# stanfordnlp/mac-network

Hardware: NVIDIA H100
Metric: mac_reasoning_steps_per_sec (higher is better)
Workload: dtype bf16

## Files before the change

mac_network_b200/csrc/read_step.cuh:

```cuda
#pragma once
#include "tc_gemm.cuh"

namespace mac {

constexpr int RS_D = 512;
constexpr int RS_BM = 64;
constexpr int RS_KB = RS_D / TC_BK;
constexpr int RS_BLK = RS_BM * TC_BK * 2;
constexpr int RS_A_BYTES = RS_KB * RS_BLK;
constexpr int RS_B_HALF = 256 * TC_BK * 2;
constexpr int RS_W_BYTES = 2 * RS_B_HALF;
constexpr int RS_STAGE = RS_W_BYTES + RS_BLK;
constexpr int RS_STAGES = 2;
constexpr int RS_Q_SLOT = RS_KB;
constexpr int RS_SLOTS = RS_Q_SLOT + 1 + RS_KB;
constexpr int RS_CONSUMERS = 256;
constexpr int RS_THREADS = RS_CONSUMERS + 32;
constexpr int RS_SMEM_BYTES = RS_A_BYTES + RS_STAGES * RS_STAGE + 1024  + 64  +
                              2 * RS_BM * 4  + 2 * RS_D * 4  +
                              2 * RS_D * 4 ;
static_assert(RS_SMEM_BYTES <= 232448, "over the sm_90 per-block shared memory opt-in limit");
static_assert(RS_STAGE % 1024 == 0 && RS_W_BYTES % 1024 == 0, "swizzled operands need 1024-byte alignment");

__device__ __forceinline__ float bf16lo(uint32_t w) { return __uint_as_float(w << 16); }
__device__ __forceinline__ float bf16hi(uint32_t w) { return __uint_as_float(w & 0xffff0000u); }

__device__ __forceinline__ void wgmma_bf16_n256(float (&d)[128], uint64_t adesc, uint64_t bdesc, uint32_t accum) {
  asm volatile(
      "{\n\t.reg .pred p;\n\t"
      "setp.ne.b32 p, %130, 0;\n\t"
      "wgmma.mma_async.sync.aligned.m64n256k16.f32.bf16.bf16 "
      "{%0, %1, %2, %3, %4, %5, %6, %7, %8, %9, %10, %11, %12, %13, %14, %15, %16, %17, %18, %19, %20, %21, %22, %23, %24, %25, %26, %27, %28, %29, %30, %31, %32, %33, %34, %35, %36, %37, %38, %39, %40, %41, %42, %43, %44, %45, %46, %47, %48, %49, %50, %51, %52, %53, %54, %55, %56, %57, %58, %59, %60, %61, %62, %63, %64, %65, %66, %67, %68, %69, %70, %71, %72, %73, %74, %75, %76, %77, %78, %79, %80, %81, %82, %83, %84, %85, %86, %87, %88, %89, %90, %91, %92, %93, %94, %95, %96, %97, %98, %99, %100, %101, %102, %103, %104, %105, %106, %107, %108, %109, %110, %111, %112, %113, %114, %115, %116, %117, %118, %119, %120, %121, %122, %123, %124, %125, %126, %127}, %128, %129, p, 1, 1, 0, 0;\n\t}"
      : "+f"(d[0]), "+f"(d[1]), "+f"(d[2]), "+f"(d[3]), "+f"(d[4]), "+f"(d[5]), "+f"(d[6]), "+f"(d[7]), "+f"(d[8]), "+f"(d[9]), "+f"(d[10]), "+f"(d[11]), "+f"(d[12]), "+f"(d[13]), "+f"(d[14]), "+f"(d[15]), "+f"(d[16]), "+f"(d[17]), "+f"(d[18]), "+f"(d[19]), "+f"(d[20]), "+f"(d[21]), "+f"(d[22]), "+f"(d[23]), "+f"(d[24]), "+f"(d[25]), "+f"(d[26]), "+f"(d[27]), "+f"(d[28]), "+f"(d[29]), "+f"(d[30]), "+f"(d[31]), "+f"(d[32]), "+f"(d[33]), "+f"(d[34]), "+f"(d[35]), "+f"(d[36]), "+f"(d[37]), "+f"(d[38]), "+f"(d[39]), "+f"(d[40]), "+f"(d[41]), "+f"(d[42]), "+f"(d[43]), "+f"(d[44]), "+f"(d[45]), "+f"(d[46]), "+f"(d[47]), "+f"(d[48]), "+f"(d[49]), "+f"(d[50]), "+f"(d[51]), "+f"(d[52]), "+f"(d[53]), "+f"(d[54]), "+f"(d[55]), "+f"(d[56]), "+f"(d[57]), "+f"(d[58]), "+f"(d[59]), "+f"(d[60]), "+f"(d[61]), "+f"(d[62]), "+f"(d[63]), "+f"(d[64]), "+f"(d[65]), "+f"(d[66]), "+f"(d[67]), "+f"(d[68]), "+f"(d[69]), "+f"(d[70]), "+f"(d[71]), "+f"(d[72]), "+f"(d[73]), "+f"(d[74]), "+f"(d[75]), "+f"(d[76]), "+f"(d[77]), "+f"(d[78]), "+f"(d[79]), "+f"(d[80]), "+f"(d[81]), "+f"(d[82]), "+f"(d[83]), "+f"(d[84]), "+f"(d[85]), "+f"(d[86]), "+f"(d[87]), "+f"(d[88]), "+f"(d[89]), "+f"(d[90]), "+f"(d[91]), "+f"(d[92]), "+f"(d[93]), "+f"(d[94]), "+f"(d[95]), "+f"(d[96]), "+f"(d[97]), "+f"(d[98]), "+f"(d[99]), "+f"(d[100]), "+f"(d[101]), "+f"(d[102]), "+f"(d[103]), "+f"(d[104]), "+f"(d[105]), "+f"(d[106]), "+f"(d[107]), "+f"(d[108]), "+f"(d[109]), "+f"(d[110]), "+f"(d[111]), "+f"(d[112]), "+f"(d[113]), "+f"(d[114]), "+f"(d[115]), "+f"(d[116]), "+f"(d[117]), "+f"(d[118]), "+f"(d[119]), "+f"(d[120]), "+f"(d[121]), "+f"(d[122]), "+f"(d[123]), "+f"(d[124]), "+f"(d[125]), "+f"(d[126]), "+f"(d[127])
      : "l"(adesc), "l"(bdesc), "r"(accum));
}
inline bool read_step_supported(int B, int N, int d) {
  return d == RS_D && N >= 1 && N <= 256 && B >= 1 && B < (1 << 22);
}

struct ReadStepParams {
  int M, N;
  const float* y;
  const float* ctrl;
  const float* bm2;
  const float* wr;
  float* logits;
};

__device__ __forceinline__ void rs_consumer_bar() { asm volatile("bar.sync 1, %0;" ::"n"(RS_CONSUMERS) : "memory"); }

__global__ void __launch_bounds__(RS_THREADS, 1)
read_step_kernel(const __grid_constant__ CUtensorMap map_p, const __grid_constant__ CUtensorMap map_q,
                 const __grid_constant__ CUtensorMap map_w1, const __grid_constant__ CUtensorMap map_w2,
                 const ReadStepParams p) {
  extern __shared__ unsigned char smem_dyn[];
  const uint32_t base_u32 = smem_u32(smem_dyn);
  unsigned char* a_tile = smem_dyn + ((1024u - (base_u32 & 1023u)) & 1023u);
  unsigned char* b_ring = a_tile + RS_A_BYTES;
  uint64_t* full = reinterpret_cast<uint64_t*>(b_ring + RS_STAGES * RS_STAGE);
  uint64_t* empty = full + RS_STAGES;
  float* s_lg = reinterpret_cast<float*>(full + 8);
  float* s_ctrl = s_lg + 2 * RS_BM;
  float* s_bm2 = s_ctrl + 2 * RS_D;
  float* s_wr = s_bm2 + RS_D;

  const int warp = threadIdx.x >> 5, lane = threadIdx.x & 31;
  const int row0 = blockIdx.x * RS_BM;
  const int s_lo = row0 / p.N;

  if (threadIdx.x == RS_CONSUMERS) {
    tma_prefetch_desc(&map_p);
    tma_prefetch_desc(&map_q);
    tma_prefetch_desc(&map_w1);
    tma_prefetch_desc(&map_w2);
    for (int i = 0; i < RS_STAGES; ++i) {
      mbar_init(&full[i], 1);
      mbar_init(&empty[i], RS_CONSUMERS / 32);
    }
    fence_mbar_init();
  }
  __syncthreads();

  if (warp == RS_CONSUMERS / 32) {
    if (elect_one()) {
      for (int j = 0; j < RS_SLOTS; ++j) {
        const int s = j % RS_STAGES;
        mbar_wait(&empty[s], ((j / RS_STAGES) & 1) ^ 1);
        unsigned char* dst = b_ring + s * RS_STAGE;
        if (j == RS_Q_SLOT) {
          mbar_expect_tx(&full[s], RS_A_BYTES);
          for (int kb = 0; kb < RS_KB; ++kb) tma_load_2d(dst + kb * RS_BLK, &map_q, kb * TC_BK, row0, &full[s]);
          continue;
        }
        const bool g1 = j < RS_Q_SLOT;
        mbar_expect_tx(&full[s], g1 ? RS_W_BYTES + RS_BLK : RS_W_BYTES);
        const CUtensorMap* m = g1 ? &map_w1 : &map_w2;
        const int k0 = (g1 ? j : j - RS_Q_SLOT - 1) * TC_BK;
        if (g1) tma_load_2d(dst + RS_W_BYTES, &map_p, k0, row0, &full[s]);
        tma_load_2d(dst, m, k0, 0, &full[s]);
        tma_load_2d(dst + RS_B_HALF, m, k0, 256, &full[s]);
      }
    }
    return;
  }

  const int tid = threadIdx.x;
  const int g = warp >> 2;
  const int rl = 16 * (warp & 3) + (lane >> 2);
  const int cq = 256 * g + 2 * (lane & 3);
  const int prow = tid >> 3;
  const int poff = prow * 128 + (tid & 7) * 16;
  const int pcol = ((tid & 7) ^ (prow & 7)) << 3;
  for (int i = tid; i < RS_D; i += RS_CONSUMERS) {
    s_bm2[i] = __ldg(p.bm2 + i);
    s_wr[i] = __ldg(p.wr + i);
  }
  float acc[128];
  const int last_row = min(p.M, row0 + RS_BM) - 1;
  const int nsamp = last_row / p.N - s_lo + 1;
  for (int q = 0; q < min(nsamp, 2); ++q)
    for (int i = tid; i < RS_D; i += RS_CONSUMERS) s_ctrl[q * RS_D + i] = __ldg(p.ctrl + (size_t)(s_lo + q) * RS_D + i);
  int yoff[2];
#pragma unroll
  for (int u = 0; u < 2; ++u) yoff[u] = min(row0 + prow + 32 * u, p.M - 1) / p.N * RS_D + pcol;

  for (int j = 0; j < RS_KB; ++j) {
    const int s = j % RS_STAGES;
    unsigned char* stage = b_ring + s * RS_STAGE;
    float4 y0[2], y1[2];
#pragma unroll
    for (int u = 0; u < 2; ++u) {
      y0[u] = *reinterpret_cast<const float4*>(p.y + yoff[u] + j * TC_BK);
      y1[u] = *reinterpret_cast<const float4*>(p.y + yoff[u] + j * TC_BK + 4);
    }
    mbar_wait(&full[s], (j / RS_STAGES) & 1);
#pragma unroll
    for (int u = 0; u < 2; ++u) {
      uint4* c = reinterpret_cast<uint4*>(stage + RS_W_BYTES + poff + u * 32 * 128);
      const uint4 v = *c;
      *c = make_uint4(pack_bf16(bf16lo(v.x) * y0[u].x, bf16hi(v.x) * y0[u].y), pack_bf16(bf16lo(v.y) * y0[u].z, bf16hi(v.y) * y0[u].w),
                      pack_bf16(bf16lo(v.z) * y1[u].x, bf16hi(v.z) * y1[u].y), pack_bf16(bf16lo(v.w) * y1[u].z, bf16hi(v.w) * y1[u].w));
    }
    fence_proxy_async();
    rs_consumer_bar();
    const uint64_t adesc = make_sw128_kmajor_desc(smem_u32(stage + RS_W_BYTES));
    const uint64_t bdesc = make_sw128_kmajor_desc(smem_u32(stage + g * RS_B_HALF));
    wgmma_fence();
#pragma unroll
    for (int k = 0; k < TC_BK / 16; ++k) wgmma_bf16_n256(acc, adesc + 2 * k, bdesc + 2 * k, (j || k) ? 1u : 0u);
    wgmma_commit();
    wgmma_wait<1>();
    wgmma_hold(acc);
    if (j && lane == 0) mbar_arrive(&empty[(j - 1) % RS_STAGES]);
  }
  wgmma_wait<0>();
  wgmma_hold(acc);
  if (lane == 0) mbar_arrive(&empty[(RS_KB - 1) % RS_STAGES]);

  constexpr int qs = RS_Q_SLOT % RS_STAGES;
  const unsigned char* q_tile = b_ring + qs * RS_STAGE;
  mbar_wait(&full[qs], (RS_Q_SLOT / RS_STAGES) & 1);
#pragma unroll
  for (int h = 0; h < 2; ++h) {
    const int r = rl + 8 * h, row = row0 + r;
#pragma unroll
    for (int j = 0; j < 32; ++j) {
      const int n = cq + 8 * j;
      const int kb = n >> 6, c = (n & 63) >> 3;
      const int off = kb * RS_BLK + r * 128 + ((c ^ (r & 7)) << 4) + (n & 7) * 2;
      const uint32_t q = *reinterpret_cast<const uint32_t*>(q_tile + off);
      const uint32_t hv = row < p.M ? pack_bf16(elu_fast(acc[4 * j + 2 * h] + bf16lo(q)), elu_fast(acc[4 * j + 2 * h + 1] + bf16hi(q)))
                                    : 0u;
      *reinterpret_cast<uint32_t*>(a_tile + off) = hv;
    }
  }
  fence_proxy_async();
  rs_consumer_bar();
  if (lane == 0) mbar_arrive(&empty[qs]);

  const uint32_t a_u = smem_u32(a_tile);
  for (int j = 0; j < RS_KB; ++j) {
    const int jj = RS_Q_SLOT + 1 + j, s = jj % RS_STAGES;
    mbar_wait(&full[s], (jj / RS_STAGES) & 1);
    const uint64_t adesc = make_sw128_kmajor_desc(a_u + j * RS_BLK);
    const uint64_t bdesc = make_sw128_kmajor_desc(smem_u32(b_ring + s * RS_STAGE + g * RS_B_HALF));
    wgmma_fence();
#pragma unroll
    for (int k = 0; k < TC_BK / 16; ++k) wgmma_bf16_n256(acc, adesc + 2 * k, bdesc + 2 * k, (j || k) ? 1u : 0u);
    wgmma_commit();
    wgmma_wait<1>();
    wgmma_hold(acc);
    if (j && lane == 0) mbar_arrive(&empty[(jj - 1) % RS_STAGES]);
  }
  wgmma_wait<0>();
  wgmma_hold(acc);
  if (lane == 0) mbar_arrive(&empty[(RS_SLOTS - 1) % RS_STAGES]);

#pragma unroll
  for (int h = 0; h < 2; ++h) {
    const int r = rl + 8 * h, row = row0 + r;
    const int s = min(row, p.M - 1) / p.N;
    const float* crow = s - s_lo < 2 ? s_ctrl + (s - s_lo) * RS_D : p.ctrl + (size_t)s * RS_D;
    float part = 0.f;
#pragma unroll
    for (int j = 0; j < 32; ++j) {
      const int n = cq + 8 * j;
      const float2 cc = *reinterpret_cast<const float2*>(crow + n);
      const float2 bb = *reinterpret_cast<const float2*>(s_bm2 + n);
      const float2 ww = *reinterpret_cast<const float2*>(s_wr + n);
      const float t0 = elu_fast((acc[4 * j + 2 * h] + bb.x) * cc.x);
      const float t1 = elu_fast((acc[4 * j + 2 * h + 1] + bb.y) * cc.y);
      part = fmaf(t0, ww.x, part);
      part = fmaf(t1, ww.y, part);
    }
    part += __shfl_xor_sync(0xffffffffu, part, 1);
    part += __shfl_xor_sync(0xffffffffu, part, 2);
    if ((lane & 3) == 0) s_lg[g * RS_BM + r] = part;
  }
  rs_consumer_bar();
  if (tid < RS_BM && row0 + tid < p.M) p.logits[row0 + tid] = s_lg[tid] + s_lg[RS_BM + tid];
}

inline int read_step_launch(const void* inv, const void* kb_bf16, const float* y, const float* control,
                            const mac_read_weights* w, float* att, float* info, int B, int N, int d, cudaStream_t stream) {
  if (!read_step_supported(B, N, d)) return MAC_ERR_UNSUPPORTED;
  if (!inv || !kb_bf16 || !y || !control || !w->Wm_bf16 || !w->Wm2_bf16 || !att || !info) return MAC_ERR_INVALID;
  const int M = B * N;
  const TcReadScratch s = tc_read_scratch(const_cast<void*>(inv), B, N, d);
  CUtensorMap mp, mq, mw1, mw2;
  int st = make_tmap_2d(&mp, s.P, 1, (uint64_t)M, (uint64_t)d, (uint64_t)d * 2, RS_BM, TC_BK, 1);
  if (st != MAC_OK) return st;
  st = make_tmap_2d(&mq, s.Q, 1, (uint64_t)M, (uint64_t)d, (uint64_t)d * 2, RS_BM, TC_BK, 1);
  if (st != MAC_OK) return st;
  st = make_tmap_2d(&mw1, w->Wm_bf16, 1, (uint64_t)d, (uint64_t)d, (uint64_t)2 * d * 2, 256, TC_BK, 1);
  if (st != MAC_OK) return st;
  st = make_tmap_2d(&mw2, w->Wm2_bf16, 1, (uint64_t)d, (uint64_t)d, (uint64_t)d * 2, 256, TC_BK, 1);
  if (st != MAC_OK) return st;
  ReadStepParams p{};
  p.M = M; p.N = N; p.y = y; p.ctrl = control; p.bm2 = w->bm2; p.wr = w->wr; p.logits = s.parts;
  MAC_CUDA_TRY(cudaFuncSetAttribute(read_step_kernel, cudaFuncAttributeMaxDynamicSharedMemorySize, RS_SMEM_BYTES));
  read_step_kernel<<<(M + RS_BM - 1) / RS_BM, RS_THREADS, RS_SMEM_BYTES, stream>>>(mp, mq, mw1, mw2, p);
  MAC_LAUNCH_CHECK();
  return mac_kb_attend_fwd(s.parts, 1, w->br, kb_bf16, 1, att, info, B, N, d, stream);
}

}
```

Measured before the change: 16540.

## Feed GEMM1 A operand from registers and add third pipeline stage

The first GEMM no longer rewrites the scaled P tile in shared memory and synchronises all consumers on a named barrier. Each warp now loads its A fragments with ldmatrix, scales them by y in registers and issues register-sourced wgmma. A third ring stage for GEMM 1 reuses the idle A-tile buffer plus an extra P block, deepening prefetch. Three producer warps release registers with setmaxnreg so consumers can hold 240 each, at the cost of more complex stage/parity bookkeeping and register pressure from double-buffered fragments.

Result: faster. 16910 (median of 6 runs) (+2.2%).

```diff
diff --git a/mac_network_b200/csrc/read_step.cuh b/mac_network_b200/csrc/read_step.cuh
--- a/mac_network_b200/csrc/read_step.cuh
+++ b/mac_network_b200/csrc/read_step.cuh
@@ -15,12 +15,19 @@
 constexpr int RS_Q_SLOT = RS_KB;
 constexpr int RS_SLOTS = RS_Q_SLOT + 1 + RS_KB;
 constexpr int RS_CONSUMERS = 256;
-constexpr int RS_THREADS = RS_CONSUMERS + 32;
-constexpr int RS_SMEM_BYTES = RS_A_BYTES + RS_STAGES * RS_STAGE + 1024  + 64  +
+constexpr int RS_THREADS = RS_CONSUMERS + 128;
+constexpr int RS_G1_STAGES = 3;
+constexpr int RS_SMEM_BYTES = RS_A_BYTES + RS_STAGES * RS_STAGE + RS_BLK  + 1024  + 64  +
                               2 * RS_BM * 4  + 2 * RS_D * 4  +
                               2 * RS_D * 4 ;
 static_assert(RS_SMEM_BYTES <= 232448, "over the sm_90 per-block shared memory opt-in limit");
 static_assert(RS_STAGE % 1024 == 0 && RS_W_BYTES % 1024 == 0, "swizzled operands need 1024-byte alignment");
+static_assert(RS_KB % RS_G1_STAGES == 2, "ring stages 0 and 1 serve equally many GEMM 1 slots");
+
+__host__ __device__ constexpr int rs_stage(int j) { return j < RS_Q_SLOT ? j % RS_G1_STAGES : (j - RS_Q_SLOT) % RS_STAGES; }
+__host__ __device__ constexpr uint32_t rs_parity(int j) {
+  return (j < RS_Q_SLOT ? j / RS_G1_STAGES : (RS_Q_SLOT + RS_G1_STAGES - 1) / RS_G1_STAGES + (j - RS_Q_SLOT) / RS_STAGES) & 1;
+}
 
 __device__ __forceinline__ float bf16lo(uint32_t w) { return __uint_as_float(w << 16); }
 __device__ __forceinline__ float bf16hi(uint32_t w) { return __uint_as_float(w & 0xffff0000u); }
@@ -34,6 +41,16 @@
       : "+f"(d[0]), "+f"(d[1]), "+f"(d[2]), "+f"(d[3]), "+f"(d[4]), "+f"(d[5]), "+f"(d[6]), "+f"(d[7]), "+f"(d[8]), "+f"(d[9]), "+f"(d[10]), "+f"(d[11]), "+f"(d[12]), "+f"(d[13]), "+f"(d[14]), "+f"(d[15]), "+f"(d[16]), "+f"(d[17]), "+f"(d[18]), "+f"(d[19]), "+f"(d[20]), "+f"(d[21]), "+f"(d[22]), "+f"(d[23]), "+f"(d[24]), "+f"(d[25]), "+f"(d[26]), "+f"(d[27]), "+f"(d[28]), "+f"(d[29]), "+f"(d[30]), "+f"(d[31]), "+f"(d[32]), "+f"(d[33]), "+f"(d[34]), "+f"(d[35]), "+f"(d[36]), "+f"(d[37]), "+f"(d[38]), "+f"(d[39]), "+f"(d[40]), "+f"(d[41]), "+f"(d[42]), "+f"(d[43]), "+f"(d[44]), "+f"(d[45]), "+f"(d[46]), "+f"(d[47]), "+f"(d[48]), "+f"(d[49]), "+f"(d[50]), "+f"(d[51]), "+f"(d[52]), "+f"(d[53]), "+f"(d[54]), "+f"(d[55]), "+f"(d[56]), "+f"(d[57]), "+f"(d[58]), "+f"(d[59]), "+f"(d[60]), "+f"(d[61]), "+f"(d[62]), "+f"(d[63]), "+f"(d[64]), "+f"(d[65]), "+f"(d[66]), "+f"(d[67]), "+f"(d[68]), "+f"(d[69]), "+f"(d[70]), "+f"(d[71]), "+f"(d[72]), "+f"(d[73]), "+f"(d[74]), "+f"(d[75]), "+f"(d[76]), "+f"(d[77]), "+f"(d[78]), "+f"(d[79]), "+f"(d[80]), "+f"(d[81]), "+f"(d[82]), "+f"(d[83]), "+f"(d[84]), "+f"(d[85]), "+f"(d[86]), "+f"(d[87]), "+f"(d[88]), "+f"(d[89]), "+f"(d[90]), "+f"(d[91]), "+f"(d[92]), "+f"(d[93]), "+f"(d[94]), "+f"(d[95]), "+f"(d[96]), "+f"(d[97]), "+f"(d[98]), "+f"(d[99]), "+f"(d[100]), "+f"(d[101]), "+f"(d[102]), "+f"(d[103]), "+f"(d[104]), "+f"(d[105]), "+f"(d[106]), "+f"(d[107]), "+f"(d[108]), "+f"(d[109]), "+f"(d[110]), "+f"(d[111]), "+f"(d[112]), "+f"(d[113]), "+f"(d[114]), "+f"(d[115]), "+f"(d[116]), "+f"(d[117]), "+f"(d[118]), "+f"(d[119]), "+f"(d[120]), "+f"(d[121]), "+f"(d[122]), "+f"(d[123]), "+f"(d[124]), "+f"(d[125]), "+f"(d[126]), "+f"(d[127])
       : "l"(adesc), "l"(bdesc), "r"(accum));
 }
+__device__ __forceinline__ void wgmma_bf16_n256_rs(float (&d)[128], uint32_t a0, uint32_t a1, uint32_t a2, uint32_t a3, uint64_t bdesc,
+                                                   uint32_t accum) {
+  asm volatile(
+      "{\n\t.reg .pred p;\n\t"
+      "setp.ne.b32 p, %133, 0;\n\t"
+      "wgmma.mma_async.sync.aligned.m64n256k16.f32.bf16.bf16 "
+      "{%0, %1, %2, %3, %4, %5, %6, %7, %8, %9, %10, %11, %12, %13, %14, %15, %16, %17, %18, %19, %20, %21, %22, %23, %24, %25, %26, %27, %28, %29, %30, %31, %32, %33, %34, %35, %36, %37, %38, %39, %40, %41, %42, %43, %44, %45, %46, %47, %48, %49, %50, %51, %52, %53, %54, %55, %56, %57, %58, %59, %60, %61, %62, %63, %64, %65, %66, %67, %68, %69, %70, %71, %72, %73, %74, %75, %76, %77, %78, %79, %80, %81, %82, %83, %84, %85, %86, %87, %88, %89, %90, %91, %92, %93, %94, %95, %96, %97, %98, %99, %100, %101, %102, %103, %104, %105, %106, %107, %108, %109, %110, %111, %112, %113, %114, %115, %116, %117, %118, %119, %120, %121, %122, %123, %124, %125, %126, %127}, {%128, %129, %130, %131}, %132, p, 1, 1, 0;\n\t}"
+      : "+f"(d[0]), "+f"(d[1]), "+f"(d[2]), "+f"(d[3]), "+f"(d[4]), "+f"(d[5]), "+f"(d[6]), "+f"(d[7]), "+f"(d[8]), "+f"(d[9]), "+f"(d[10]), "+f"(d[11]), "+f"(d[12]), "+f"(d[13]), "+f"(d[14]), "+f"(d[15]), "+f"(d[16]), "+f"(d[17]), "+f"(d[18]), "+f"(d[19]), "+f"(d[20]), "+f"(d[21]), "+f"(d[22]), "+f"(d[23]), "+f"(d[24]), "+f"(d[25]), "+f"(d[26]), "+f"(d[27]), "+f"(d[28]), "+f"(d[29]), "+f"(d[30]), "+f"(d[31]), "+f"(d[32]), "+f"(d[33]), "+f"(d[34]), "+f"(d[35]), "+f"(d[36]), "+f"(d[37]), "+f"(d[38]), "+f"(d[39]), "+f"(d[40]), "+f"(d[41]), "+f"(d[42]), "+f"(d[43]), "+f"(d[44]), "+f"(d[45]), "+f"(d[46]), "+f"(d[47]), "+f"(d[48]), "+f"(d[49]), "+f"(d[50]), "+f"(d[51]), "+f"(d[52]), "+f"(d[53]), "+f"(d[54]), "+f"(d[55]), "+f"(d[56]), "+f"(d[57]), "+f"(d[58]), "+f"(d[59]), "+f"(d[60]), "+f"(d[61]), "+f"(d[62]), "+f"(d[63]), "+f"(d[64]), "+f"(d[65]), "+f"(d[66]), "+f"(d[67]), "+f"(d[68]), "+f"(d[69]), "+f"(d[70]), "+f"(d[71]), "+f"(d[72]), "+f"(d[73]), "+f"(d[74]), "+f"(d[75]), "+f"(d[76]), "+f"(d[77]), "+f"(d[78]), "+f"(d[79]), "+f"(d[80]), "+f"(d[81]), "+f"(d[82]), "+f"(d[83]), "+f"(d[84]), "+f"(d[85]), "+f"(d[86]), "+f"(d[87]), "+f"(d[88]), "+f"(d[89]), "+f"(d[90]), "+f"(d[91]), "+f"(d[92]), "+f"(d[93]), "+f"(d[94]), "+f"(d[95]), "+f"(d[96]), "+f"(d[97]), "+f"(d[98]), "+f"(d[99]), "+f"(d[100]), "+f"(d[101]), "+f"(d[102]), "+f"(d[103]), "+f"(d[104]), "+f"(d[105]), "+f"(d[106]), "+f"(d[107]), "+f"(d[108]), "+f"(d[109]), "+f"(d[110]), "+f"(d[111]), "+f"(d[112]), "+f"(d[113]), "+f"(d[114]), "+f"(d[115]), "+f"(d[116]), "+f"(d[117]), "+f"(d[118]), "+f"(d[119]), "+f"(d[120]), "+f"(d[121]), "+f"(d[122]), "+f"(d[123]), "+f"(d[124]), "+f"(d[125]), "+f"(d[126]), "+f"(d[127])
+      : "r"(a0), "r"(a1), "r"(a2), "r"(a3), "l"(bdesc), "r"(accum));
+}
 inline bool read_step_supported(int B, int N, int d) {
   return d == RS_D && N >= 1 && N <= 256 && B >= 1 && B < (1 << 22);
 }
@@ -47,6 +64,19 @@
   float* logits;
 };
 
+__device__ __forceinline__ void ldmatrix_x4(uint32_t* r, uint32_t addr) {
+  asm volatile("ldmatrix.sync.aligned.m8n8.x4.shared.b16 {%0, %1, %2, %3}, [%4];"
+               : "=r"(r[0]), "=r"(r[1]), "=r"(r[2]), "=r"(r[3]) : "r"(addr) : "memory");
+}
+__device__ __forceinline__ uint32_t scale_bf16x2(uint32_t v, float2 y) { return pack_bf16(bf16lo(v) * y.x, bf16hi(v) * y.y); }
+__device__ __forceinline__ void frag_hold(uint32_t (&a)[16]) {
+#pragma unroll
+  for (int i = 0; i < 16; ++i) asm volatile("" : "+r"(a[i])::"memory");
+}
+
+__device__ __forceinline__ void rs_producer_regs() { asm volatile("setmaxnreg.dec.sync.aligned.u32 24;" ::: "memory"); }
+__device__ __forceinline__ void rs_consumer_regs() { asm volatile("setmaxnreg.inc.sync.aligned.u32 240;" ::: "memory"); }
+
 __device__ __forceinline__ void rs_consumer_bar() { asm volatile("bar.sync 1, %0;" ::"n"(RS_CONSUMERS) : "memory"); }
 
 __global__ void __launch_bounds__(RS_THREADS, 1)
@@ -57,8 +87,9 @@
   const uint32_t base_u32 = smem_u32(smem_dyn);
   unsigned char* a_tile = smem_dyn + ((1024u - (base_u32 & 1023u)) & 1023u);
   unsigned char* b_ring = a_tile + RS_A_BYTES;
-  uint64_t* full = reinterpret_cast<uint64_t*>(b_ring + RS_STAGES * RS_STAGE);
-  uint64_t* empty = full + RS_STAGES;
+  unsigned char* p_extra = b_ring + RS_STAGES * RS_STAGE;
+  uint64_t* full = reinterpret_cast<uint64_t*>(p_extra + RS_BLK);
+  uint64_t* empty = full + RS_G1_STAGES;
   float* s_lg = reinterpret_cast<float*>(full + 8);
   float* s_ctrl = s_lg + 2 * RS_BM;
   float* s_bm2 = s_ctrl + 2 * RS_D;
@@ -73,7 +104,7 @@
     tma_prefetch_desc(&map_q);
     tma_prefetch_desc(&map_w1);
     tma_prefetch_desc(&map_w2);
-    for (int i = 0; i < RS_STAGES; ++i) {
+    for (int i = 0; i < RS_G1_STAGES; ++i) {
       mbar_init(&full[i], 1);
       mbar_init(&empty[i], RS_CONSUMERS / 32);
     }
@@ -81,12 +112,13 @@
   }
   __syncthreads();
 
-  if (warp == RS_CONSUMERS / 32) {
-    if (elect_one()) {
+  if (warp >= RS_CONSUMERS / 32) {
+    rs_producer_regs();
+    if (warp == RS_CONSUMERS / 32 && elect_one()) {
       for (int j = 0; j < RS_SLOTS; ++j) {
-        const int s = j % RS_STAGES;
-        mbar_wait(&empty[s], ((j / RS_STAGES) & 1) ^ 1);
-        unsigned char* dst = b_ring + s * RS_STAGE;
+        const int s = rs_stage(j);
+        mbar_wait(&empty[s], rs_parity(j) ^ 1);
+        unsigned char* dst = s < RS_STAGES ? b_ring + s * RS_STAGE : a_tile;
         if (j == RS_Q_SLOT) {
           mbar_expect_tx(&full[s], RS_A_BYTES);
           for (int kb = 0; kb < RS_KB; ++kb) tma_load_2d(dst + kb * RS_BLK, &map_q, kb * TC_BK, row0, &full[s]);
@@ -96,7 +128,7 @@
         mbar_expect_tx(&full[s], g1 ? RS_W_BYTES + RS_BLK : RS_W_BYTES);
         const CUtensorMap* m = g1 ? &map_w1 : &map_w2;
         const int k0 = (g1 ? j : j - RS_Q_SLOT - 1) * TC_BK;
-        if (g1) tma_load_2d(dst + RS_W_BYTES, &map_p, k0, row0, &full[s]);
+        if (g1) tma_load_2d(s < RS_STAGES ? dst + RS_W_BYTES : p_extra, &map_p, k0, row0, &full[s]);
         tma_load_2d(dst, m, k0, 0, &full[s]);
         tma_load_2d(dst + RS_B_HALF, m, k0, 256, &full[s]);
       }
@@ -104,13 +136,11 @@
     return;
   }
 
+  rs_consumer_regs();
   const int tid = threadIdx.x;
   const int g = warp >> 2;
   const int rl = 16 * (warp & 3) + (lane >> 2);
   const int cq = 256 * g + 2 * (lane & 3);
-  const int prow = tid >> 3;
-  const int poff = prow * 128 + (tid & 7) * 16;
-  const int pcol = ((tid & 7) ^ (prow & 7)) << 3;
   for (int i = tid; i < RS_D; i += RS_CONSUMERS) {
     s_bm2[i] = __ldg(p.bm2 + i);
     s_wr[i] = __ldg(p.wr + i);
@@ -120,46 +150,57 @@
   const int nsamp = last_row / p.N - s_lo + 1;
   for (int q = 0; q < min(nsamp, 2); ++q)
     for (int i = tid; i < RS_D; i += RS_CONSUMERS) s_ctrl[q * RS_D + i] = __ldg(p.ctrl + (size_t)(s_lo + q) * RS_D + i);
-  int yoff[2];
-#pragma unroll
-  for (int u = 0; u < 2; ++u) yoff[u] = min(row0 + prow + 32 * u, p.M - 1) / p.N * RS_D + pcol;
-
+  const int yoff_a = min(row0 + rl, p.M - 1) / p.N * RS_D, yoff_b = min(row0 + rl + 8, p.M - 1) / p.N * RS_D;
+  const uint32_t frag_row = (uint32_t)(16 * (warp & 3) + (lane & 7) + 8 * ((lane >> 3) & 1)) * 128u;
+  uint32_t af[2][16];
+
+  float2 ya[8], yb[8];
+#pragma unroll
+  for (int i = 0; i < 8; ++i) {
+    ya[i] = *reinterpret_cast<const float2*>(p.y + yoff_a + 8 * i + 2 * (lane & 3));
+    yb[i] = *reinterpret_cast<const float2*>(p.y + yoff_b + 8 * i + 2 * (lane & 3));
+  }
+#pragma unroll
   for (int j = 0; j < RS_KB; ++j) {
-    const int s = j % RS_STAGES;
-    unsigned char* stage = b_ring + s * RS_STAGE;
-    float4 y0[2], y1[2];
-#pragma unroll
-    for (int u = 0; u < 2; ++u) {
-      y0[u] = *reinterpret_cast<const float4*>(p.y + yoff[u] + j * TC_BK);
-      y1[u] = *reinterpret_cast<const float4*>(p.y + yoff[u] + j * TC_BK + 4);
-    }
-    mbar_wait(&full[s], (j / RS_STAGES) & 1);
-#pragma unroll
-    for (int u = 0; u < 2; ++u) {
-      uint4* c = reinterpret_cast<uint4*>(stage + RS_W_BYTES + poff + u * 32 * 128);
-      const uint4 v = *c;
-      *c = make_uint4(pack_bf16(bf16lo(v.x) * y0[u].x, bf16hi(v.x) * y0[u].y), pack_bf16(bf16lo(v.y) * y0[u].z, bf16hi(v.y) * y0[u].w),
-                      pack_bf16(bf16lo(v.z) * y1[u].x, bf16hi(v.z) * y1[u].y), pack_bf16(bf16lo(v.w) * y1[u].z, bf16hi(v.w) * y1[u].w));
-    }
-    fence_proxy_async();
-    rs_consumer_bar();
-    const uint64_t adesc = make_sw128_kmajor_desc(smem_u32(stage + RS_W_BYTES));
+    const int s = rs_stage(j);
+    uint32_t (&a)[16] = af[j & 1];
+    mbar_wait(&full[s], rs_parity(j));
+    unsigned char* stage = s < RS_STAGES ? b_ring + s * RS_STAGE : a_tile;
+    const uint32_t pf = smem_u32(s < RS_STAGES ? stage + RS_W_BYTES : p_extra) + frag_row;
+#pragma unroll
+    for (int kk = 0; kk < TC_BK / 16; ++kk) {
+      ldmatrix_x4(a + 4 * kk, pf + (((2 * kk + (lane >> 4)) ^ (lane & 7)) << 4));
+      a[4 * kk + 0] = scale_bf16x2(a[4 * kk + 0], ya[2 * kk]);
+      a[4 * kk + 1] = scale_bf16x2(a[4 * kk + 1], yb[2 * kk]);
+      a[4 * kk + 2] = scale_bf16x2(a[4 * kk + 2], ya[2 * kk + 1]);
+      a[4 * kk + 3] = scale_bf16x2(a[4 * kk + 3], yb[2 * kk + 1]);
+    }
+    if (j + 1 < RS_KB) {
+#pragma unroll
+      for (int i = 0; i < 8; ++i) {
+        ya[i] = *reinterpret_cast<const float2*>(p.y + yoff_a + (j + 1) * TC_BK + 8 * i + 2 * (lane & 3));
+        yb[i] = *reinterpret_cast<const float2*>(p.y + yoff_b + (j + 1) * TC_BK + 8 * i + 2 * (lane & 3));
+      }
+    }
     const uint64_t bdesc = make_sw128_kmajor_desc(smem_u32(stage + g * RS_B_HALF));
     wgmma_fence();
 #pragma unroll
-    for (int k = 0; k < TC_BK / 16; ++k) wgmma_bf16_n256(acc, adesc + 2 * k, bdesc + 2 * k, (j || k) ? 1u : 0u);
+    for (int kk = 0; kk < TC_BK / 16; ++kk)
+      wgmma_bf16_n256_rs(acc, a[4 * kk], a[4 * kk + 1], a[4 * kk + 2], a[4 * kk + 3], bdesc + 2 * kk, (j || kk) ? 1u : 0u);
     wgmma_commit();
     wgmma_wait<1>();
     wgmma_hold(acc);
-    if (j && lane == 0) mbar_arrive(&empty[(j - 1) % RS_STAGES]);
+    if (j) frag_hold(af[(j - 1) & 1]);
+    if (j && lane == 0) mbar_arrive(&empty[rs_stage(j - 1)]);
   }
   wgmma_wait<0>();
   wgmma_hold(acc);
-  if (lane == 0) mbar_arrive(&empty[(RS_KB - 1) % RS_STAGES]);
-
-  constexpr int qs = RS_Q_SLOT % RS_STAGES;
+  frag_hold(af[(RS_KB - 1) & 1]);
+  if (lane == 0) mbar_arrive(&empty[rs_stage(RS_KB - 1)]);
+
+  constexpr int qs = rs_stage(RS_Q_SLOT);
   const unsigned char* q_tile = b_ring + qs * RS_STAGE;
-  mbar_wait(&full[qs], (RS_Q_SLOT / RS_STAGES) & 1);
+  mbar_wait(&full[qs], rs_parity(RS_Q_SLOT));
 #pragma unroll
   for (int h = 0; h < 2; ++h) {
     const int r = rl + 8 * h, row = row0 + r;
@@ -180,8 +221,8 @@
 
   const uint32_t a_u = smem_u32(a_tile);
   for (int j = 0; j < RS_KB; ++j) {
-    const int jj = RS_Q_SLOT + 1 + j, s = jj % RS_STAGES;
-    mbar_wait(&full[s], (jj / RS_STAGES) & 1);
+    const int jj = RS_Q_SLOT + 1 + j, s = rs_stage(jj);
+    mbar_wait(&full[s], rs_parity(jj));
     const uint64_t adesc = make_sw128_kmajor_desc(a_u + j * RS_BLK);
     const uint64_t bdesc = make_sw128_kmajor_desc(smem_u32(b_ring + s * RS_STAGE + g * RS_B_HALF));
     wgmma_fence();
@@ -190,11 +231,11 @@
     wgmma_commit();
     wgmma_wait<1>();
     wgmma_hold(acc);
-    if (j && lane == 0) mbar_arrive(&empty[(jj - 1) % RS_STAGES]);
+    if (j && lane == 0) mbar_arrive(&empty[rs_stage(jj - 1)]);
   }
   wgmma_wait<0>();
   wgmma_hold(acc);
-  if (lane == 0) mbar_arrive(&empty[(RS_SLOTS - 1) % RS_STAGES]);
+  if (lane == 0) mbar_arrive(&empty[rs_stage(RS_SLOTS - 1)]);
 
 #pragma unroll
   for (int h = 0; h < 2; ++h) {
```
